# jambo6/online-neural-cdes

Hardware: AMD Instinct MI355X
Metric: solved integration steps/sec (fwd+adjoint) (higher is better)
Workload: dtype f32; 1 GPU; BASELINE cfg2: rectilinear interpolation, rk4 step 1, B=4096 per GPU (global 4096), raw L=200 -> T=399 knots, C=20, H=HH=32, nl=3; step = forward + adjoint backward + Adam; global_batch=4096, seq_len=200, parallelism=dp1

## Files before the change

### online-neural-cdes_amd/csrc/ncde_coop.h

```cpp
#pragma once
#include "ncde_bf3.h"
#include "ncde_common.h"

#define COOP_NRT 5
#define COOP_RPM (4 * COOP_NRT)
#define COOP_NCH 4
#define COOP_SPIN_LIMIT (1 << 22)

namespace {

typedef unsigned u32x2c __attribute__((ext_vector_type(2)));
typedef _Float16 h16x4 __attribute__((ext_vector_type(4)));

struct CoopDims {
    int H, C, dlast, M, G;
    __host__ __device__ int xl() const { return dlast * 16; }
    __host__ __device__ int off_as() const { return xl(); }
    __host__ __device__ int off_dx() const { return off_as() + H * 16; }
    __host__ __device__ int off_sc() const { return off_dx() + C * 16; }
    __host__ __device__ int off_ko() const { return off_sc() + 64; }
    __host__ __device__ int off_part() const { return off_ko() + H * 16; }
    __host__ __device__ long long per_tile() const { return (long long)off_part() + (long long)M * dlast * 16; }
    __host__ __device__ long long per_tile_fwd() const { return (long long)off_part(); }
};

__device__ __forceinline__ __amdgpu_buffer_rsrc_t coop_rsrc(const void* p) {
    return __builtin_amdgcn_make_buffer_rsrc(const_cast<void*>(p), 0, 0x7ffffffc, 0x00020000);
}
__device__ __forceinline__ void coop_st16(__amdgpu_buffer_rsrc_t r, float* base, bool same, long long float_off, u32x4 v) {
    if (same) *reinterpret_cast<u32x4*>(base + float_off) = v;
    else __builtin_amdgcn_raw_buffer_store_b128(v, r, (int)(float_off * 4), 0, 16);
}
__device__ __forceinline__ void coop_st4(__amdgpu_buffer_rsrc_t r, float* base, bool same, long long float_off, float v) {
    if (same) base[float_off] = v;
    else __builtin_amdgcn_raw_buffer_store_b32(__float_as_uint(v), r, (int)(float_off * 4), 0, 16);
}
__device__ __forceinline__ u32x4 coop_ld16(__amdgpu_buffer_rsrc_t r, long long float_off) {
    return __builtin_amdgcn_raw_buffer_load_b128(r, (int)(float_off * 4), 0, 16);
}
__device__ __forceinline__ float coop_ld4(__amdgpu_buffer_rsrc_t r, long long float_off) {
    return __uint_as_float(__builtin_amdgcn_raw_buffer_load_b32(r, (int)(float_off * 4), 0, 16));
}
__device__ __forceinline__ f32x4 coop_ld16f(__amdgpu_buffer_rsrc_t r, long long float_off) {
    return __builtin_bit_cast(f32x4, coop_ld16(r, float_off));
}

__device__ __forceinline__ float coop_pow2_scale(float m) {
    if (!(m > 0.0f) || !(m < 3.0e38f)) return 1.0f;
    int e = (int)((__float_as_uint(m) >> 23) & 255u) - 126;
    e = e < -100 ? -100 : (e > 100 ? 100 : e);
    return __uint_as_float((unsigned)(127 - e) << 23);
}
__device__ __forceinline__ float coop_pow2_inv(float s) { return __uint_as_float((254u - ((__float_as_uint(s) >> 23) & 255u)) << 23); }

struct CoopSync {
    unsigned* words;
    int G;
    unsigned* status;
    unsigned spin;
};
__device__ __forceinline__ void coop_give_up(const CoopSync& sy) {
    __hip_atomic_store(sy.words + sy.G, 1u, __ATOMIC_RELAXED, __HIP_MEMORY_SCOPE_AGENT);
    __hip_atomic_store(sy.status, 1u, __ATOMIC_RELAXED, __HIP_MEMORY_SCOPE_AGENT);
}
__host__ __device__ inline int coop_sync_words(int G, int n_tiles) { return 2 * G + 1 + n_tiles; }
__device__ __forceinline__ void coop_arrive(const CoopSync& sy, int g) {
    __hip_atomic_fetch_add(sy.words + g, 1u, __ATOMIC_RELAXED, __HIP_MEMORY_SCOPE_AGENT);
}
__device__ __forceinline__ bool coop_wait(const CoopSync& sy, int g, unsigned target, int* flag_lds, int tid) {
    if (tid == 0) {
        int ok = 1;
        unsigned spins = 0;
// ... 146 lines not shown
```

### online-neural-cdes_amd/csrc/ncde_dwo2.hip

```cpp
#include "ncde_common.h"
#include "ncde_bf3.h"
#define NCDE_COOP_NO_KERNELS
#include "ncde_coop.h"
#include "ncde_dwo2.h"

template <int NRT>
__device__ __forceinline__ void dwo_h2_body(const KArgs& a, int n_sc, int n_st, float* gpartB) {
    extern __shared__ __attribute__((aligned(16))) float lds[];
    constexpr int dlast = 128, PK = 8, NCH = 4, NWV = 16 / NRT;
    const int tid = threadIdx.x, lane = tid & 63;
    const int wave = __builtin_amdgcn_readfirstlane(tid >> 6);
    const int li = lane & 15, lk = lane >> 4;
    const int C = a.C, H = a.H, ncq = C >> 2;
    const int n_pair = n_st >> 1, parts = a.dw2_parts, nrg = gridDim.x / parts;
    int bx_, by_;
    if ((parts & 7) == 0) {
        const int xcd = blockIdx.x & 7, slot = blockIdx.x >> 3;
        by_ = xcd * (parts >> 3) + slot / nrg;
        bx_ = slot % nrg;
    } else {
        by_ = blockIdx.x / nrg;
        bx_ = blockIdx.x % nrg;
    }
    const int bx = __builtin_amdgcn_readfirstlane(bx_), by = __builtin_amdgcn_readfirstlane(by_);
    const int nRC = H >> 4, nRD = (C + 15) >> 4;
    const int oXP = 2 * 2048, oRC = oXP + 4096, oRD = oRC + 2 * nRC * 256, oS = oRD + 2 * nRD * 256, per_buf = oS + 2 * 256;
    int hb[NRT], cq[NRT];
    u32x4 W[NRT][NCH][2];
    float bias[NRT];
    f32x4 gW[NRT][PK];
    float gb[NRT];
#pragma unroll
    for (int q = 0; q < NRT; ++q) {
        const int rt = (bx * NWV + wave) * NRT + q;
        hb[q] = rt / ncq;
        cq[q] = rt - hb[q] * ncq;
        const int mem = rt / COOP_RPM, rw = (rt % COOP_RPM) / COOP_NRT, qq = rt % COOP_NRT;
        const unsigned* wp = a.coop_img + (long long)mem * (coop_p_words() + coop_t_words()) + rw * (40 * 64 * 4);
#pragma unroll
        for (int c = 0; c < NCH; ++c)
#pragma unroll
            for (int pc = 0; pc < 2; ++pc) W[q][c][pc] = *reinterpret_cast<const u32x4*>(wp + ((((qq * 4 + c) * 2 + pc) * 64) + lane) * 4);
        bias[q] = a.bo[(4 * hb[q] + (li >> 2)) * C + 4 * cq[q] + (li & 3)];
#pragma unroll
        for (int jt = 0; jt < PK; ++jt) gW[q][jt] = (f32x4){0.f, 0.f, 0.f, 0.f};
        gb[q] = 0.0f;
    }
    const float sigma = coop_pow2_scale(__uint_as_float(*a.win_max)), inv_sigma = coop_pow2_inv(sigma);
    const int my_n = by < n_pair ? (n_pair - by + parts - 1) / parts : 0;
    typedef const __attribute__((address_space(1))) void* gptr_t;
    typedef __attribute__((address_space(3))) void* lptr_t;
    const int n_chunk = 2 * 8 + 16 + 2 * nRC + 2 * nRD + 2;
#ifndef DW2_NIW
#define DW2_NIW 4
#endif
    constexpr int NIW = DW2_NIW < NWV ? DW2_NIW : NWV;
    constexpr int NSLOT = (60 + NIW - 1) / NIW;
    long long s_const[NSLOT];
    int s_sc[NSLOT], s_pr[NSLOT], s_lds[NSLOT];
#pragma unroll
    for (int j = 0; j < NSLOT; ++j) {
        int k = wave + NIW * j;
        if (k >= n_chunk) k = wave < NIW ? wave : 0;
        long long cst;
        int ssc, spr, sl;
        if (k < 16) { cst = (long long)(k >> 3) * 2048 + (k & 7) * 256; ssc = n_st * 2048; spr = 2 * 2048; sl = k * 256; }
        else if ((k -= 16) < 16) { cst = (a.recB - a.recA) + (long long)k * 256; ssc = n_pair * 4096; spr = 4096; sl = oXP + k * 256; }
        else if ((k -= 16) < 2 * nRC) { const int t2 = k >= nRC ? 1 : 0, kk = k - t2 * nRC; cst = (a.recC - a.recA) + (long long)t2 * (H * 16) + kk * 256; ssc = n_st * H * 16; spr = 2 * H * 16; sl = oRC + k * 256; }
        else if ((k -= 2 * nRC) < 2 * nRD) { const int t2 = k >= nRD ? 1 : 0, kk = k - t2 * nRD; cst = (a.recD - a.recA) + (long long)t2 * (C * 16) + kk * 256; ssc = n_st * C * 16; spr = 2 * C * 16; sl = oRD + k * 256; }
        else { k -= 2 * nRD; cst = (a.recS - a.recA) + (long long)k * 32; ssc = n_st * 32; spr = 64; sl = oS + k * 256; }
        s_const[j] = cst; s_sc[j] = ssc; s_pr[j] = spr; s_lds[j] = sl;
    }
    const int my_n_ = by < n_pair ? (n_pair - by + parts - 1) / parts : 0;
    long long s_off[NSLOT];
    int s_dpr[NSLOT], s_dsc[NSLOT];
#pragma unroll
    for (int j = 0; j < NSLOT; ++j) {
        s_off[j] = s_const[j] + (long long)by * s_pr[j];
        s_dpr[j] = parts * s_pr[j];
        s_dsc[j] = s_sc[j] - (my_n_ - 1) * parts * s_pr[j];
    }
    auto issue = [&](bool wrap, int buf) {
        if (wave >= NIW) return;
#pragma unroll
        for (int j = 0; j < NSLOT; ++j) {
            __builtin_amdgcn_global_load_lds((gptr_t)(a.recA + s_off[j] + lane * 4), (lptr_t)(lds + buf * per_buf + s_lds[j]), 16, 0, 0);
            s_off[j] += wrap ? s_dsc[j] : s_dpr[j];
        }
    };
#ifdef NCDE_DW2_PROF
    unsigned long long dprof[5] = {0, 0, 0, 0, 0}, dlast_ = __builtin_readcyclecounter();
#define DW2_TICK(k) { const unsigned long long n_ = __builtin_readcyclecounter(); dprof[k] += n_ - dlast_; dlast_ = n_; }
#else
#define DW2_TICK(k)
#endif
    u32x4 Ap[NRT][2];
    auto p_and_epilogue = [&](int buf, int lane, int li, int lk) {
        const float* B_ = lds + buf * per_buf;
        const unsigned* XS = reinterpret_cast<const unsigned*>(B_);
        auto ldx = [&](int t2, int c, int pc) { return *reinterpret_cast<const u32x4*>(XS + t2 * 2048 + ((c * 2 + pc) * 64 + lane) * 4); };
        constexpr bool AHEAD = NRT == 4;
        u32x4 nx0, nx1;
        if constexpr (AHEAD) { nx0 = ldx(0, 0, 0); nx1 = ldx(0, 0, 1); }
#pragma unroll
        for (int t2 = 0; t2 < 2; ++t2) {
            const float* S_ = B_ + oS + t2 * 256;
            const f32x4 isx4 = *reinterpret_cast<const f32x4*>(S_ + 4 * lk);
            f32x4 isx2;
#pragma unroll
            for (int r = 0; r < 4; ++r) isx2[r] = isx4[r] * NCDE_TANH_PRESCALE;
            const float fT = sigma * S_[17];
            auto lda = [&](int i) { return *reinterpret_cast<const f32x4*>(B_ + oRC + t2 * nRC * 256 + (4 * hb[i] + (li >> 2)) * 16 + 4 * lk); };
            auto ldd = [&](int i) { return *reinterpret_cast<const f32x4*>(B_ + oRD + t2 * nRD * 256 + (4 * cq[i] + (li & 3)) * 16 + 4 * lk); };
            f32x4 na4, nd4;
            if constexpr (AHEAD) { na4 = lda(0); nd4 = ldd(0); }
            f32x4 pm[NRT], px[NRT];
#pragma unroll
            for (int i = 0; i < NRT; ++i) {
#pragma unroll
                for (int r = 0; r < 4; ++r) pm[i][r] = bias[i] * coop_pow2_inv(isx4[r]);
                px[i] = (f32x4){0.f, 0.f, 0.f, 0.f};
            }
#pragma unroll
            for (int c = 0; c < NCH; ++c) {
                u32x4 x0, x1;
                if constexpr (AHEAD) {
                    x0 = nx0; x1 = nx1;
                    if (c + 1 < NCH) { nx0 = ldx(t2, c + 1, 0); nx1 = ldx(t2, c + 1, 1); }
                    else if (t2 == 0) { nx0 = ldx(1, 0, 0); nx1 = ldx(1, 0, 1); }
                } else { x0 = ldx(t2, c, 0); x1 = ldx(t2, c, 1); }
#pragma unroll
                for (int i = 0; i < NRT; ++i) px[i] = mfma_h(x0, W[i][c][1], px[i]);
#pragma unroll
                for (int i = 0; i < NRT; ++i) pm[i] = mfma_h(x0, W[i][c][0], pm[i]);
#pragma unroll
                for (int i = 0; i < NRT; ++i) px[i] = mfma_h(x1, W[i][c][0], px[i]);
            }
#pragma unroll
            for (int i = 0; i < NRT; ++i) {
                const f32x4 pc = h2_combine(pm[i], px[i]);
                f32x4 a4, d4;
                if constexpr (AHEAD) {
                    a4 = na4; d4 = nd4;
                    if (i + 1 < NRT) { na4 = lda(i + 1); nd4 = ldd(i + 1); }
                } else { a4 = lda(i); d4 = ldd(i); }
                float dps[4];
#pragma unroll
                for (int r = 0; r < 4; ++r) {
                    const float th = tanh_prescaled(pc[r] * isx2[r]);
                    const float dp = (a4[r] * d4[r]) * (1.0f - th * th);
                    gb[i] += dp;
                    dps[r] = dp * fT;
                }
                unsigned h0, l0, h1, l1;
                coop_split2(dps[0], dps[1], h0, l0);
                coop_split2(dps[2], dps[3], h1, l1);
                Ap[i][0][2 * t2] = h0; Ap[i][0][2 * t2 + 1] = h1;
                Ap[i][1][2 * t2] = l0; Ap[i][1][2 * t2 + 1] = l1;
            }
        }
    };
    auto dwo_products = [&](int buf, int lane) {
        const unsigned* XP = reinterpret_cast<const unsigned*>(lds + buf * per_buf + oXP);
        constexpr bool AHEAD = NRT == 4;
        auto ldb = [&](int jt, int pc) { return *reinterpret_cast<const u32x4*>(XP + ((jt * 2 + pc) * 64 + lane) * 4); };
        u32x4 nb0, nb1;
        if constexpr (AHEAD) { nb0 = ldb(0, 0); nb1 = ldb(0, 1); }
        f32x4 ptx[NRT];
#pragma unroll
        for (int jt = 0; jt < PK; ++jt) {
            u32x4 b0, b1;
            if constexpr (AHEAD) {
                b0 = nb0; b1 = nb1;
                if (jt + 1 < PK) { nb0 = ldb(jt + 1, 0); nb1 = ldb(jt + 1, 1); }
            } else { b0 = ldb(jt, 0); b1 = ldb(jt, 1); }
            f32x4 tx[NRT];
#pragma unroll
            for (int i = 0; i < NRT; ++i) tx[i] = mfma_h(Ap[i][0], b1, (f32x4){0.f, 0.f, 0.f, 0.f});
#pragma unroll
            for (int i = 0; i < NRT; ++i) gW[i][jt] = mfma_h(Ap[i][0], b0, gW[i][jt]);
#pragma unroll
            for (int i = 0; i < NRT; ++i) tx[i] = mfma_h(Ap[i][1], b0, tx[i]);
            if (jt > 0) {
#pragma unroll
                for (int i = 0; i < NRT; ++i) gW[i][jt - 1] = h2_combine(gW[i][jt - 1], ptx[i]);
            }
#pragma unroll
            for (int i = 0; i < NRT; ++i) ptx[i] = tx[i];
        }
#pragma unroll
        for (int i = 0; i < NRT; ++i) gW[i][PK - 1] = h2_combine(gW[i][PK - 1], ptx[i]);
    };
    if (my_n > 0 && n_sc > 0) {
        const int nq = n_sc * my_n;
        int k_n = 0;
        issue(k_n + 1 == my_n, 0);
        if (++k_n == my_n) k_n = 0;
        asm volatile("s_waitcnt vmcnt(0)" ::: "memory");
        __syncthreads();
        for (int q = 0; q < nq; ++q) {
            const int buf = q & 1;
            if (q + 1 < nq) {
                issue(k_n + 1 == my_n, buf ^ 1);
                if (++k_n == my_n) k_n = 0;
            }
            __builtin_amdgcn_sched_barrier(0);
            DW2_TICK(0)
            int t_ = tid;
            asm volatile("" : "+v"(t_));
            const int lane_ = t_ & 63, li_ = t_ & 15, lk_ = (t_ >> 4) & 3;
            p_and_epilogue(buf, lane_, li_, lk_);
            DW2_TICK(1)
            dwo_products(buf, lane_);
            DW2_TICK(2)
            __builtin_amdgcn_sched_barrier(0);
            asm volatile("s_waitcnt vmcnt(0)" ::: "memory");
            DW2_TICK(3)
            __syncthreads();
            DW2_TICK(4)
        }
#ifdef NCDE_DW2_PROF
        if (lane == 0)
            for (int k = 0; k < 5; ++k) a.grad_z0[((long long)blockIdx.x * NWV + wave) * 8 + k] = (float)dprof[k] / (float)nq;
#endif
    }
    const long long wo_sz = (long long)H * C * dlast, theta_o = wo_sz + (long long)H * C;
    float* gp = gpartB + (long long)by * theta_o;
#pragma unroll
    for (int q = 0; q < NRT; ++q) {
#pragma unroll
        for (int jt = 0; jt < PK; ++jt)
#pragma unroll
            for (int r = 0; r < 4; ++r) {
                float* dst = gp + ((long long)(4 * hb[q] + lk) * C + 4 * cq[q] + r) * dlast + 16 * jt + li;
                const float v = gW[q][jt][r] * inv_sigma;
                *dst = a.dw2_accum ? *dst + v : v;
            }
        float v = gb[q];
        v += __shfl_xor(v, 16, 64); v += __shfl_xor(v, 32, 64);
        if (lk == 0) {
            float* dst = gp + wo_sz + (4 * hb[q] + (li >> 2)) * C + 4 * cq[q] + (li & 3);
            *dst = a.dw2_accum ? *dst + v : v;
        }
    }
}

extern "C" __global__ __launch_bounds__(512) void ncde_dwo_h2(KArgs a, int n_sc, int n_st, float* gpartB) { dwo_h2_body<2>(a, n_sc, n_st, gpartB); }
```

### online-neural-cdes_amd/csrc/ncde_tiled.hip

```cpp
#include <type_traits>
#include "ncde_common.h"
#include "ncde_bf3.h"
#include "ncde_host.h"
#include "ncde_tiled.h"
#include "ncde_coop.h"
#include "ncde_dwo2.h"

#define TL_NW 8
#define TL_THREADS (64 * TL_NW)
#define TL_EMAX 16

namespace {

template <int NS, int NT, bool QUINTIC = true>
__device__ __forceinline__ void tl_load_dx(const KArgs& a, int b0, int idx, float frac, float kdt, float* DX, int tid) {
    constexpr int NSP = NS * 16;
    const int C = a.C, Cc = a.Cc;
    for (int e = tid; e < NSP * C; e += NT) {
        const int s = e / C, c = e - s * C;
        const int b = b0 + s;
        float v = 0.0f;
        if (b < a.B && c < Cc) {
            const float* p = a.coeffs + (long long)b * a.cs_b + (long long)idx * a.cs_t;
            if (a.interp == NCDE_INTERP_LINEAR) {
// ... 676 lines not shown
            const float v = live ? a.z0[(long long)b * a.Hr + u] : 0.0f;
            y0[q] = v;
            YS[e] = v;
            if (live) a.out[((long long)b * a.n_out) * a.Hr + u] = v;
        }
    }
    const int S = n_stages(a.method);
    const int dlast = a.dout[a.n_layers - 1];
    const int nkb_o = dlast >> 4;
    Panel<RESH ? RESH : 1> wf[2];
    f32x4 bfv[2];
    if constexpr (RESH != 0) {
        const int li = lane & 15, lk = lane >> 4;
        int l1 = 0;
        for (int l = 1; l < a.n_layers; ++l)
            if (a.W[l] != a.W[0]) { l1 = l; break; }
#pragma unroll
        for (int sl = 0; sl < 2; ++sl) {
            const int l = sl == 0 ? 0 : l1;
            const int tw = wave < RESH ? wave : 0;
            wf[sl] = tl_load_panel<RESH ? RESH : 1>(a.W[l] + (long long)(16 * tw + li) * (16 * RESH) + 4 * lk, 0);
            bfv[sl] = *reinterpret_cast<const f32x4*>(a.b[l] + 16 * tw + 4 * lk);
        }
    }
    int cur_idx = -1;
    const bool planned = a.plan != nullptr;
    if (planned && !plan_header_ok(a, S)) return;
    const int n_steps = planned ? a.n_steps_fwd : a.T - 1;
    const int* pout = planned ? a.plan + plan_off_out(S, a.n_steps_fwd) : nullptr;
    int sc = 0;
#ifdef NCDE_TL_PROF
    unsigned long long fprof[8] = {0, 0, 0, 0, 0, 0, 0, 0}, flast = __builtin_readcyclecounter();
    unsigned long long kprof[3] = {0, 0, 0}, klast = 0;
#endif
    for (int n = 0; n < n_steps; ++n) {
        const int* pstep = planned ? a.plan + plan_off_fwd() + n * plan_step_words(S) : nullptr;
        const float dt = planned ? __int_as_float(pstep[0]) : 1.0f;
        for (int j = 0; j < S; ++j, ++sc) {
            const StageDesc sd = planned ? plan_stage(pstep, j) : default_stage(a.method, (float)n + stage_offset(a.method, j), a.n_pieces);
            const int idx = sd.idx;
            bool dx_new = false;
            if constexpr (DIRECT != 0) {
                tl_load_cin<NS, NT>(a, b0, sd, a.field_input == NCDE_INPUT_EVALUATE, YS, H, tid);
            } else if (a.interp != NCDE_INTERP_LINEAR || idx != cur_idx) {
                tl_load_dx<NS, NT, COOP == 0>(a, b0, idx, sd.frac, sd.kdt, DX, tid);
                cur_idx = idx;
                dx_new = true;
            }
            __syncthreads();
            if constexpr (COOP != 0) {
                if (dx_new) {
                    const long long my_base = (long long)blockIdx.x * cd.per_tile_fwd();
                    for (int e = tid; e < a.C * NSP / 4; e += NT) coop_st16(crs, a.coop_x, c_same, my_base + cd.off_dx() + e * 4, *reinterpret_cast<const u32x4*>(DX + e * 4));
                }
            }
            if (a.stages) {
                const int Hr = a.Hr;
                float* rec = a.stages + ((long long)(n * S + j) * (a.Brec ? a.Brec : a.B) + b0) * Hr;
                for (int e = tid; e < NSP * Hr; e += NT) {
                    const int s = e / Hr, u = e - s * Hr;
                    if (b0 + s < a.B) rec[e] = YS[((u >> 2) * NSP + s) * 4 + (u & 3)];
                }
            }
            FW_TICK(0)
            const float* in = YS;
            for (int l = 0; l < a.n_layers; ++l) {
                float* outb = (l & 1) ? ACT1 : ACT0;
                if constexpr (RESH != 0) {
                    if (wave < RESH) {
                        const int li = lane & 15, lk = lane >> 4;
                        const bool s0 = a.W[l] == a.W[0];
                        f32x4 acc[1];
                        acc[0] = s0 ? bfv[0] : bfv[1];
                        if (s0) tl_mma_panel<1, RESH ? RESH : 1>(wf[0], in, 0, li, lk, acc);
                        else tl_mma_panel<1, RESH ? RESH : 1>(wf[1], in, 0, li, lk, acc);
                        f32x4 o;
#pragma unroll
                        for (int r = 0; r < 4; ++r) o[r] = relu_dev(acc[0][r]);
                        *reinterpret_cast<f32x4*>(outb + ((4 * wave + lk) * NSP + li) * 4) = o;
                        if constexpr (BF != 0) {
                            if (l == a.n_layers - 1) {
                                typedef unsigned u32x2 __attribute__((ext_vector_type(2)));
                                if constexpr (BF == 2) {
                                    unsigned h0, l0, h1, l1;
                                    split_pair_h(o[0], o[1], h0, l0, mx);
                                    split_pair_h(o[2], o[3], h1, l1, mx);
                                    unsigned* dst = XB + ((((wave >> 1) * 2) * 4 + 2 * (wave & 1) + (lk >> 1)) * 16 + li) * 4 + 2 * (lk & 1);
                                    *reinterpret_cast<u32x2*>(dst) = (u32x2){h0, h1};
                                    *reinterpret_cast<u32x2*>(dst + 256) = (u32x2){l0, l1};
                                } else {
                                    unsigned h0, m0, l0, h1, m1, l1;
                                    split_pair(o[0], o[1], h0, m0, l0);
                                    split_pair(o[2], o[3], h1, m1, l1);
                                    unsigned* dst = XB + ((((wave >> 1) * 3) * 4 + 2 * (wave & 1) + (lk >> 1)) * 16 + li) * 4 + 2 * (lk & 1);
                                    *reinterpret_cast<u32x2*>(dst) = (u32x2){h0, h1};
                                    *reinterpret_cast<u32x2*>(dst + 256) = (u32x2){m0, m1};
                                    *reinterpret_cast<u32x2*>(dst + 512) = (u32x2){l0, l1};
                                }
                            }
                        }
                    }
                } else {
                    const TlW wr_ = tl_wref(lds, DIRECT != 0 ? a.tres[l] : 0, a.W[l], a.b[l], a.dout[l], a.din[l]);
                    if constexpr (COOP != 0)
                        tl_dense_relu<NS, NWV, 0, 0, 4>(wr_.W, wr_.b, a.dout[l], a.din[l], in, outb, wave, lane, nullptr, wr_.ld);
                    else if constexpr (BF == 2)
                        tl_dense_relu<NS, NWV, 0, 1>(wr_.W, wr_.b, a.dout[l], a.din[l], in, outb, wave, lane,
                                                     l == a.n_layers - 1 ? XB : nullptr, wr_.ld, &mx);
                    else
                        tl_dense_relu<NS, NWV>(wr_.W, wr_.b, a.dout[l], a.din[l], in, outb, wave, lane,
                                               (BF != 0 && l == a.n_layers - 1) ? XB : nullptr, wr_.ld);
                }
                __syncthreads();
                in = outb;
            }
            FW_TICK(1)
            float* KG = in == ACT0 ? ACT1 : ACT0;
            if constexpr (DIRECT != 0) {
                const TlW wo_ = tl_wref(lds, a.tres_o, a.Wo, a.bo, H, dlast);
                tl_dense_relu<NS, NWV, 1>(wo_.W, wo_.b, H, dlast, in, KO, wave, lane, nullptr, wo_.ld);
                if constexpr (GATED != 0) {
                    const TlW wg_ = tl_wref(lds, a.tres_g, a.Wg, a.bg, H, dlast);
                    tl_dense_relu<NS, NWV, 2>(wg_.W, wg_.b, H, dlast, in, KG, wave, lane, nullptr, wg_.ld);
                }
            } else
            if constexpr (COOP != 0) {
                const int li = lane & 15, lk = lane >> 4, C = a.C;
                const long long my_base = (long long)blockIdx.x * cd.per_tile_fwd();
                const unsigned bar1 = (2u * (unsigned)sc + 1u) * (unsigned)cd.M, bar2 = bar1 + (unsigned)cd.M;
                {
                    float mxl = 0.0f;
                    for (int e = tid; e < 128 * NSP; e += NT) mxl = fmaxf(mxl, fabsf(in[e]));
                    mxl = fmaxf(mxl, __shfl_xor(mxl, 1, 64)); mxl = fmaxf(mxl, __shfl_xor(mxl, 2, 64));
                    if ((lane & 3) == 0) CMX[wave * 16 + ((lane >> 2) & 15)] = mxl;
                }
                __syncthreads();
                if (tid < 16) {
                    float m_ = 0.0f;
#pragma unroll
                    for (int wv = 0; wv < 8; ++wv) m_ = fmaxf(m_, CMX[wv * 16 + tid]);
                    const float sx = coop_pow2_scale(m_), isx = coop_pow2_inv(sx) * a.coop_scale[1];
                    CSG[tid] = sx; CSG[16 + tid] = isx;
                    coop_st4(crs, a.coop_x, c_same, my_base + cd.off_sc() + tid, sx); coop_st4(crs, a.coop_x, c_same, my_base + cd.off_sc() + 16 + tid, isx);
                }
                __syncthreads();
                if (wave < 4) {
                    const int c = wave, ub = 32 * c + 8 * lk;
                    const f32x4 v0 = *reinterpret_cast<const f32x4*>(in + (((ub >> 2)) * NSP + li) * 4);
                    const f32x4 v1 = *reinterpret_cast<const f32x4*>(in + (((ub >> 2) + 1) * NSP + li) * 4);
                    const float sx = CSG[li];
                    unsigned h[4], l[4];
                    coop_split2(v0[0] * sx, v0[1] * sx, h[0], l[0]); coop_split2(v0[2] * sx, v0[3] * sx, h[1], l[1]);
                    coop_split2(v1[0] * sx, v1[1] * sx, h[2], l[2]); coop_split2(v1[2] * sx, v1[3] * sx, h[3], l[3]);
                    coop_st16(crs, a.coop_x, c_same, my_base + ((c * 2 + 0) * 64 + lane) * 4, (u32x4){h[0], h[1], h[2], h[3]});
                    coop_st16(crs, a.coop_x, c_same, my_base + ((c * 2 + 1) * 64 + lane) * 4, (u32x4){l[0], l[1], l[2], l[3]});
                }
                asm volatile("s_waitcnt vmcnt(0)" ::: "memory");
                __syncthreads();
                if (tid == 0 && !(a.coop_inject != 0 && blockIdx.x == 1 && sc == 0)) coop_arrive(csy, c_grp);
                FW_TICK(2)
                auto poison = [&]() {
                    const float qnan = __builtin_nanf("");
                    for (long long e = tid; e < (long long)NSP * a.n_out * a.Hr; e += NT)
                        if (b0 + (int)(e / ((long long)a.n_out * a.Hr)) < a.B) a.out[(long long)b0 * a.n_out * a.Hr + e] = qnan;
                };
                if (!coop_wait(csy, c_grp, bar1, CFL, tid)) { poison(); return; }
                FW_TICK(3)
                const int ncq = C >> 2, jh = COOP_RPM / ncq, wph = 4 / jh;
                const int rw = wave & 3, half_w = wave >> 2;
                const int cq0 = (c_mem * COOP_RPM + rw * COOP_NRT) % ncq;
                const int n_dx4 = C * NSP / 4, n_it = cd.M / 2;
                typedef const __attribute__((address_space(1))) void* gptr_t;
                typedef __attribute__((address_space(3))) void* lptr_t;
                const int n_dxw = (n_dx4 + 63) >> 6;
                auto stage_load = [&](int it_, int buf, int tid) {
                    const int wv = __builtin_amdgcn_readfirstlane(tid >> 6), w64 = wv * 64;
#pragma unroll
                    for (int hf = 0; hf < 2; ++hf) {
                        const float* src = a.coop_x + (long long)(c_grp + cd.G * (2 * it_ + hf)) * cd.per_tile_fwd();
                        __builtin_amdgcn_global_load_lds((gptr_t)(src + tid * 4), (lptr_t)(CBX + (buf * 2 + hf) * 2048 + w64 * 4), 16, 0, 16);
                        if (wv < n_dxw) __builtin_amdgcn_global_load_lds((gptr_t)(src + cd.off_dx() + tid * 4), (lptr_t)(CDX + (buf * 2 + hf) * 1280 + w64 * 4), 16, 0, 16);
                        else if (wv == 6 && tid < 400)
                            __builtin_amdgcn_global_load_lds((gptr_t)(src + cd.off_sc() + (tid - 384) * 4), (lptr_t)(CSC + (buf * 2 + hf) * 64), 16, 0, 16);
                    }
                };
                stage_load(0, 0, tid);
                asm volatile("s_waitcnt vmcnt(0)" ::: "memory");
                __syncthreads();
                const int tid_outer = tid;
#ifdef NCDE_TL_PROF
                klast = __builtin_readcyclecounter();
#endif
                for (int it = 0; it <= n_it; ++it) {
                    int tid = tid_outer;
                    asm volatile("" : "+v"(tid));
                    const int lane = tid & 63, li = tid & 15, lk = (tid >> 4) & 3;
                    const int buf = it & 1;
                    if (it + 1 < n_it) stage_load(it + 1, buf ^ 1, tid);
                    if (it < n_it) {
                        const float* bxs = CBX + (buf * 2 + half_w) * 2048;
                        const float isx = CSC[(buf * 2 + half_w) * 64 + 16 + li];
                        const float sxw = coop_pow2_inv(isx);
                        const float isx2 = isx * NCDE_TANH_PRESCALE;
                        float kk = 0.0f;
                        auto wfr = [&](int k) -> u32x4 {
                            if (k < FWD_KREG) return cw.f[k];
                            return *reinterpret_cast<const u32x4*>(CWL + ((rw * (40 - FWD_KREG) + (k - FWD_KREG)) * 64 + lane) * 4);
                        };
                        auto p_batch = [&](auto q0c, auto nqc) {
                            constexpr int Q0 = decltype(q0c)::value, NQ = decltype(nqc)::value;
                            f32x4 pm[NQ], px[NQ];
#pragma unroll
                            for (int i = 0; i < NQ; ++i) {
                                const f32x4 bsv = *reinterpret_cast<const f32x4*>(CBO + ((rw * COOP_NRT + Q0 + i) * 4 + lk) * 4);
#pragma unroll
                                for (int r = 0; r < 4; ++r) pm[i][r] = bsv[r] * sxw;
                                px[i] = (f32x4){0.f, 0.f, 0.f, 0.f};
                            }
                            u32x4 b0_ = *reinterpret_cast<const u32x4*>(bxs + lane * 4), b1_ = *reinterpret_cast<const u32x4*>(bxs + (64 + lane) * 4);
#pragma unroll
                            for (int c = 0; c < COOP_NCH; ++c) {
                                const u32x4 c0_ = b0_, c1_ = b1_;
                                if (c + 1 < COOP_NCH) {
                                    b0_ = *reinterpret_cast<const u32x4*>(bxs + (((c + 1) * 2 + 0) * 64 + lane) * 4);
                                    b1_ = *reinterpret_cast<const u32x4*>(bxs + (((c + 1) * 2 + 1) * 64 + lane) * 4);
                                }
#pragma unroll
                                for (int i = 0; i < NQ; ++i) pm[i] = mfma_h(wfr(((Q0 + i) * 4 + c) * 2 + 0), c0_, pm[i]);
#pragma unroll
                                for (int i = 0; i < NQ; ++i) px[i] = mfma_h(wfr(((Q0 + i) * 4 + c) * 2 + 1), c0_, px[i]);
#pragma unroll
                                for (int i = 0; i < NQ; ++i) px[i] = mfma_h(wfr(((Q0 + i) * 4 + c) * 2 + 0), c1_, px[i]);
                            }
#pragma unroll
                            for (int i = 0; i < NQ; ++i) {
                                const f32x4 pc4 = h2_combine(pm[i], px[i]);
                                const f32x4 dxv = *reinterpret_cast<const f32x4*>(CDX + (buf * 2 + half_w) * 1280 + ((cq0 + Q0 + i) * NSP + li) * 4);
#pragma unroll
                                for (int r = 0; r < 4; ++r) kk = fmaf(tanh_prescaled(pc4[r] * isx2), dxv[r], kk);
                            }
                        };
                        if ((wave & 1) == 0) {
                            p_batch(std::integral_constant<int, 0>{}, std::integral_constant<int, 3>{});
                            p_batch(std::integral_constant<int, 3>{}, std::integral_constant<int, 2>{});
                        } else {
                            p_batch(std::integral_constant<int, 3>{}, std::integral_constant<int, 2>{});
                            p_batch(std::integral_constant<int, 0>{}, std::integral_constant<int, 3>{});
                        }
                        CKX[(buf * 8 + wave) * 64 + lane] = kk;
                    }
                    if (it >= 1 && tid < 2 * 64 * jh) {
                        const int hf = tid / (64 * jh), hl = (tid >> 6) % jh, ln = tid & 63, pb = buf ^ 1;
                        float ksum = 0.0f;
                        for (int wv = hl * wph; wv < (hl + 1) * wph; ++wv) ksum += CKX[(pb * 8 + 4 * hf + wv) * 64 + ln];
                        const long long tb = (long long)(c_grp + cd.G * (2 * (it - 1) + hf)) * cd.per_tile_fwd();
                        coop_st4(crs, a.coop_x, c_same, tb + cd.off_ko() + ((c_mem * jh + hl) * NSP + (ln & 15)) * 4 + (ln >> 4), ksum);
                    }
#ifdef NCDE_TL_PROF
                    { const unsigned long long n_ = __builtin_readcyclecounter(); kprof[0] += n_ - klast; klast = n_; }
#endif
                    if (it + 1 < n_it) asm volatile("s_waitcnt vmcnt(0)" ::: "memory");
#ifdef NCDE_TL_PROF
                    { const unsigned long long n_ = __builtin_readcyclecounter(); kprof[1] += n_ - klast; klast = n_; }
#endif
                    __syncthreads();
#ifdef NCDE_TL_PROF
                    { const unsigned long long n_ = __builtin_readcyclecounter(); kprof[2] += n_ - klast; klast = n_; }
#endif
                }
                asm volatile("s_waitcnt vmcnt(0)" ::: "memory");
                __syncthreads();
                FW_TICK(4)
                if (tid == 0) coop_arrive(csy, c_grp);
                if (!coop_wait(csy, c_grp, bar2, CFL, tid)) { poison(); return; }
                FW_TICK(5)
                for (int e4 = tid * 4; e4 < HS; e4 += NT * 4) *reinterpret_cast<f32x4*>(KO + e4) = coop_ld16f(crs, my_base + cd.off_ko() + e4);
            } else
            if constexpr (BF == 2) {
                switch (nkb_o) {
                    case 8: tl_output_h2<4, NWV, GATED>(a, XB, DX, KO, wave, lane); break;
                    case 4: tl_output_h2<2, NWV, GATED>(a, XB, DX, KO, wave, lane); break;
                    default: tl_output_h2<1, NWV, GATED>(a, XB, DX, KO, wave, lane); break;
                }
            } else if constexpr (BF != 0) {
                switch (nkb_o) {
                    case 8: tl_output_bf<4, NWV, GATED>(a, XB, DX, KO, wave, lane); break;
                    case 4: tl_output_bf<2, NWV, GATED>(a, XB, DX, KO, wave, lane); break;
                    default: tl_output_bf<1, NWV, GATED>(a, XB, DX, KO, wave, lane); break;
                }
            } else
            switch (nkb_o) {
                case 8: tl_output_whole<NS, 8, NWV, GATED>(a, in, DX, KO, wave, lane); break;
                case 4: tl_output_whole<NS, 4, NWV, GATED>(a, in, DX, KO, wave, lane); break;
                case 2: tl_output_whole<NS, 2, NWV, GATED>(a, in, DX, KO, wave, lane); break;
                case 1: tl_output_whole<NS, 1, NWV, GATED>(a, in, DX, KO, wave, lane); break;
// ... 444 lines not shown
        }
    }

    Panel<PK> wf[2];
    f32x4 bfv[2];
    float wb[2][4 * PK];
    WoTile<PK> wo[2];
    if constexpr (RES != 0) {
        const int li = lane & 15, lk = lane >> 4;
        int l1 = 0;
        for (int l = 1; l < L; ++l)
            if (a.gW_off[l] != a.gW_off[0]) { l1 = l; break; }
        const int K = dlast;
#pragma unroll
        for (int sl = 0; sl < 2; ++sl) {
            const int l = sl == 0 ? 0 : l1;
            const int tw = wave < PK ? wave : 0;
            wf[sl] = tl_load_panel<PK>(a.W[l] + (long long)(16 * tw + li) * K + 4 * lk, 0);
            bfv[sl] = *reinterpret_cast<const f32x4*>(a.b[l] + 16 * tw + 4 * lk);
#pragma unroll
            for (int kb = 0; kb < PK; ++kb)
#pragma unroll
                for (int e = 0; e < 4; ++e) wb[sl][4 * kb + e] = a.W[l][(long long)(16 * kb + 4 * lk + e) * K + 16 * tw + li];
        }
        if constexpr (RES == 1) {
            const int nhb = H >> 2, ncq = C >> 2;
#pragma unroll
            for (int q = 0; q < 2; ++q) {
                int hb = wave + NWV * (q / ncq), cq = q % ncq;
                if (hb >= nhb) { hb = 0; cq = 0; }
                wo[q].P = tl_load_panel<PK>(a.Wo + (long long)((4 * hb + (li >> 2)) * C + 4 * cq + (li & 3)) * dlast + 4 * lk, 0);
                wo[q].bias = *reinterpret_cast<const f32x4*>(a.bo + (4 * hb + lk) * C + 4 * cq);
            }
        }
    }

    CoopWeights cw;
    CoopDims cd{};
    CoopSync csy{};
    __amdgpu_buffer_rsrc_t crs = coop_rsrc(a.coop_x);
    int c_grp = 0, c_mem = 0, c_hbw = 0;
    bool c_same = false;
    float* const CDP = SC;
    float* const CBX = CDP + 2 * 10 * 2 * 64 * 4;
    float* const CDX = CBX + 2 * 8 * 64 * 4;
    float* const CAS = CDX + 2 * 80 * 16;
    float* const CSC = CAS + 2 * 256;
    float* const CKX = CSC + 2 * 64;
    float* const CIS = CKX + 2 * 4 * 64;
    int* const CFL = reinterpret_cast<int*>(CIS + 2 * 16);
    float* const CBO = reinterpret_cast<float*>(XBA) + 2048;
    float* const CMX = CDP;
    float* const CSG = CDP + 3 * 8 * 16;
    if constexpr (COOP != 0) {
        cd.H = H; cd.C = C; cd.dlast = dlast; cd.M = a.coop_M; cd.G = a.coop_G;
        csy.words = a.coop_sync; csy.G = a.coop_G; csy.status = a.coop_status; csy.spin = a.coop_spin;
        c_grp = blockIdx.x % a.coop_G;
        c_mem = blockIdx.x / a.coop_G;
        c_hbw = (c_mem * COOP_RPM + (wave & 3) * COOP_NRT) / (C >> 2);
        coop_load_weights<0, COOP_PIN>(cw, a.coop_img, c_mem, wave, lane);
        const int same = coop_same_xcd(csy, c_grp, c_mem, a.coop_M, (int)gridDim.x, CFL, tid);
        if (same < 0) return;
        c_same = same != 0;
    }

    constexpr int DXMAXC = NWV == 8 ? 80 : 160;
    constexpr int DXE = (NSP * DXMAXC + NT - 1) / NT, YSE = TL_EADJ;
    float dxn[DXE], ysn[YSE];
    const bool wide_c = C > DXMAXC;
    StageDesc sdn;
    const float* recn = nullptr;
    auto stage_desc = [&](int n, int j) {
        if (planned) return plan_stage(step_of(n), disc ? S - 1 - j : j);
        return default_stage(a.method, disc ? (float)(n - 1) + stage_offset(a.method, S - 1 - j) : -(-(float)n + stage_offset(a.method, j)), a.n_pieces);
    };
    auto dx_value = [&](int e, const StageDesc& sd) {
        const int idx = sd.idx;
        const float frac = sd.frac, kdt = sd.kdt;
        float v = 0.0f;
        const int s = e / C, c = e - s * C, b = b0 + s;
        const int Cc = a.Cc;
        if (b < a.B && c < Cc) {
            const float* cp = a.coeffs + (long long)b * a.cs_b + (long long)idx * a.cs_t;
            const bool value = DIRECT != 0 && a.field_input == NCDE_INPUT_EVALUATE;
            if (a.interp == NCDE_INTERP_LINEAR) {
                v = cp[a.cs_t + c] - cp[c];
                if (value) v = cp[c] + (frac * v) / kdt;
                else if (kdt != 1.0f) v = v / kdt;
            } else if (COOP == 0 && a.interp == NCDE_INTERP_QUINTIC) {
                v = quintic_eval(cp + c, Cc, frac, value);
            } else {
                const float bb = cp[Cc + c], cc = cp[2 * Cc + c], dd = cp[3 * Cc + c];
                if (value) {
                    float inner = 0.5f * cc + (dd * frac) / 3.0f;
                    inner = bb + inner * frac;
                    v = cp[c] + inner * frac;
                } else {
                    const float inner = cc + dd * frac;
                    v = bb + inner * frac;
                }
            }
        }
        return v;
    };
    auto prefetch = [&](int n, int j) {
        sdn = stage_desc(n, j);
// ... 138 lines not shown
                    }
                    for (int e = tid; e < H * NSP; e += NT) {
                        const int hh = e >> 4, s = e & 15;
                        rc[e] = w * AS[((hh >> 2) * NSP + s) * 4 + (hh & 3)];
                    }
                    for (int e = tid; e < C * NSP; e += NT) rd[e] = DX[e];
            };
            if constexpr (DIRECT != 0) {
                float* DPT = G0;
                float* SG = SC;
                const TlW wo_ = tl_wref(lds, a.tres_o, a.Wo, a.bo, H, dlast);
                const TlW wg_ = tl_wref(lds, GATED != 0 ? a.tres_g : 0, a.Wg, a.bg, H, dlast);
                tl_dense_relu<1, NWV, 1>(wo_.W, wo_.b, H, dlast, in, KOY, wave, lane, nullptr, wo_.ld);
                if constexpr (GATED != 0) tl_dense_relu<1, NWV, 2>(wg_.W, wg_.b, H, dlast, in, SG, wave, lane, nullptr, wg_.ld);
                __syncthreads();
                for (int e = tid; e < HS; e += NT) {
                    const float th = KOY[e], dm = AS[e];
                    if constexpr (GATED != 0) {
                        const float sg = SG[e];
                        KOY[e] = sg * th;
                        DPT[e] = (dm * sg) * (1.0f - th * th);
                        SG[e] = (dm * th) * (sg * (1.0f - sg));
                    } else {
                        DPT[e] = dm * (1.0f - th * th);
                    }
                }
                __syncthreads();
                if (w != 0.0f) {
                    tl_dw_acc<NWV, TL_DWT>(DPT, in, H, dlast, w, dwo, wave, lane);
                    if constexpr (GATED != 0) tl_dw_acc<NWV, TL_DWT>(SG, in, H, dlast, w, dwg, wave, lane);
                    if (tid < H) {
                        float sum = 0.0f, sumg = 0.0f;
#pragma unroll
                        for (int s = 0; s < NSP; ++s) {
                            sum += DPT[((tid >> 2) * NSP + s) * 4 + (tid & 3)];
                            if constexpr (GATED != 0) sumg += SG[((tid >> 2) * NSP + s) * 4 + (tid & 3)];
                        }
                        dbo += w * sum;
                        dbg += w * sumg;
                    }
                }
                tl_hidden_bwd<NWV>(wo_.W, H, dlast, DPT, in, true, G1, wave, lane, GATED != 0 ? wg_.W : nullptr, GATED != 0 ? SG : nullptr, wo_.ld);
                __syncthreads();
            } else {
                if constexpr (COOP != 0) {
                    const int li = lane & 15, lk = lane >> 4;
                    const long long my_base = (long long)blockIdx.x * cd.per_tile();
                    const unsigned bar1 = (2u * (unsigned)sc + 1u) * (unsigned)cd.M, bar2 = bar1 + (unsigned)cd.M;
                    {
                        float mx = 0.0f, ma = 0.0f, md = 0.0f;
                        for (int e = tid; e < dlast * NSP; e += NT) mx = fmaxf(mx, fabsf(in[e]));
                        for (int e = tid; e < HS; e += NT) ma = fmaxf(ma, fabsf(AS[e]));
                        for (int e = tid; e < C * NSP; e += NT) md = fmaxf(md, fabsf(DX[e]));
                        mx = fmaxf(mx, __shfl_xor(mx, 1, 64)); mx = fmaxf(mx, __shfl_xor(mx, 2, 64));
                        ma = fmaxf(ma, __shfl_xor(ma, 1, 64)); ma = fmaxf(ma, __shfl_xor(ma, 2, 64));
                        md = fmaxf(md, __shfl_xor(md, 1, 64)); md = fmaxf(md, __shfl_xor(md, 2, 64));
                        if ((lane & 3) == 0) {
                            const int s_ = (lane >> 2) & 15;
                            CMX[(0 * 8 + wave) * 16 + s_] = mx; CMX[(1 * 8 + wave) * 16 + s_] = ma; CMX[(2 * 8 + wave) * 16 + s_] = md;
                        }
                    }
                    __syncthreads();
                    if (tid < 16) {
                        float m3[3];
#pragma unroll
                        for (int k = 0; k < 3; ++k) {
                            float m_ = 0.0f;
#pragma unroll
                            for (int wv = 0; wv < 8; ++wv) m_ = fmaxf(m_, CMX[(k * 8 + wv) * 16 + tid]);
                            m3[k] = m_;
                        }
                        const float sw_inv = a.coop_scale[1];
                        const float sx = coop_pow2_scale(m3[0]), sd = coop_pow2_scale(m3[1] * m3[2]);
                        const float isx = coop_pow2_inv(sx) * sw_inv, isd = coop_pow2_inv(sd) * sw_inv;
                        CSG[tid] = sx; CSG[16 + tid] = isx; CSG[32 + tid] = sd; CSG[48 + tid] = isd;
                        coop_st4(crs, a.coop_x, c_same, my_base + cd.off_sc() + tid, sx); coop_st4(crs, a.coop_x, c_same, my_base + cd.off_sc() + 16 + tid, isx);
                        coop_st4(crs, a.coop_x, c_same, my_base + cd.off_sc() + 32 + tid, sd); coop_st4(crs, a.coop_x, c_same, my_base + cd.off_sc() + 48 + tid, isd);
                        float mt = m3[0], bt = fabsf(w) * (m3[1] * m3[2]);
#pragma unroll
                        for (int o = 8; o > 0; o >>= 1) { mt = fmaxf(mt, __shfl_xor(mt, o, 64)); bt = fmaxf(bt, __shfl_xor(bt, o, 64)); }
                        const float uT = coop_pow2_scale(mt), iuT = coop_pow2_inv(uT);
                        float* rs = a.recS + ((long long)sc * n_st + blockIdx.x) * 32;
                        rs[tid] = isx;
                        if (tid == 0) {
                            CSG[64] = uT;
                            rs[16] = uT; rs[17] = iuT;
                            const float bq = bt * iuT;
                            if (bq > 0.0f && bq < 3.0e38f) atomicMax(a.win_max, __float_as_uint(bq));
                        }
                    }
                    __syncthreads();
                    if (wave < 4) {
                        const int c = wave, ub = 32 * c + 8 * lk;
                        const f32x4 v0 = *reinterpret_cast<const f32x4*>(in + (((ub >> 2)) * NSP + li) * 4);
                        const f32x4 v1 = *reinterpret_cast<const f32x4*>(in + (((ub >> 2) + 1) * NSP + li) * 4);
                        const float sx = CSG[li];
                        unsigned h[4], l[4];
                        coop_split2(v0[0] * sx, v0[1] * sx, h[0], l[0]); coop_split2(v0[2] * sx, v0[3] * sx, h[1], l[1]);
                        coop_split2(v1[0] * sx, v1[1] * sx, h[2], l[2]); coop_split2(v1[2] * sx, v1[3] * sx, h[3], l[3]);
                        coop_st16(crs, a.coop_x, c_same, my_base + ((c * 2 + 0) * 64 + lane) * 4, (u32x4){h[0], h[1], h[2], h[3]});
                        coop_st16(crs, a.coop_x, c_same, my_base + ((c * 2 + 1) * 64 + lane) * 4, (u32x4){l[0], l[1], l[2], l[3]});
                    }
                    {
                        for (int e = tid; e < HS / 4; e += NT) coop_st16(crs, a.coop_x, c_same, my_base + cd.off_as() + e * 4, *reinterpret_cast<const u32x4*>(AS + e * 4));
                        for (int e = tid; e < C * NSP / 4; e += NT) coop_st16(crs, a.coop_x, c_same, my_base + cd.off_dx() + e * 4, *reinterpret_cast<const u32x4*>(DX + e * 4));
                    }
                    asm volatile("s_waitcnt vmcnt(0)" ::: "memory");
                    __syncthreads();
                    if (tid == 0 && !(a.coop_inject != 0 && blockIdx.x == 1 && sc == 0 && a.resume == 0)) coop_arrive(csy, c_grp);
                    TL_TICK(8)
                    coop_load_weights<COOP_PIN, 40>(cw, a.coop_img, c_mem, wave, lane);
                    {
                        const long long tile = (long long)sc * n_st + blockIdx.x;
                        if (wave < 4) {
                            const int c = wave, ub = 32 * c + 8 * lk;
                            const f32x4 v0 = *reinterpret_cast<const f32x4*>(in + (((ub >> 2)) * NSP + li) * 4);
                            const f32x4 v1 = *reinterpret_cast<const f32x4*>(in + (((ub >> 2) + 1) * NSP + li) * 4);
                            const float sx = CSG[li];
                            unsigned h[4], l[4];
                            coop_split2(v0[0] * sx, v0[1] * sx, h[0], l[0]); coop_split2(v0[2] * sx, v0[3] * sx, h[1], l[1]);
                            coop_split2(v1[0] * sx, v1[1] * sx, h[2], l[2]); coop_split2(v1[2] * sx, v1[3] * sx, h[3], l[3]);
                            unsigned* ra = reinterpret_cast<unsigned*>(a.recA) + tile * 2048;
                            *reinterpret_cast<u32x4*>(ra + ((c * 2 + 0) * 64 + lane) * 4) = (u32x4){h[0], h[1], h[2], h[3]};
                            *reinterpret_cast<u32x4*>(ra + ((c * 2 + 1) * 64 + lane) * 4) = (u32x4){l[0], l[1], l[2], l[3]};
                        }
                        {
                            const float uT = CSG[64];
                            unsigned* rbp = reinterpret_cast<unsigned*>(a.recB) + ((long long)sc * (n_st >> 1) + (blockIdx.x >> 1)) * 4096;
                            const int half = blockIdx.x & 1;
                            for (int e = tid; e < 128 * 4; e += NT) {
                                const int k = e >> 2, kg = e & 3, ln = (k & 15) + 16 * kg;
                                float v[4];
#pragma unroll
                                for (int q = 0; q < 4; ++q) v[q] = in[((k >> 2) * NSP + 4 * kg + q) * 4 + (k & 3)] * uT;
                                unsigned h0, l0, h1, l1;
                                coop_split2(v[0], v[1], h0, l0);
                                coop_split2(v[2], v[3], h1, l1);
                                unsigned* dst = rbp + (((k >> 4) * 2) * 64 + ln) * 4 + 2 * half;
                                *reinterpret_cast<u32x2c*>(dst) = (u32x2c){h0, h1};
// ... 1706 lines not shown
```

Measured before the change: 195.1 million sample-steps/s.

## Skip MFMA work for zero channel quads when dx is narrow (rectilinear)

Detects at runtime whether the control-path increments are nonzero only in the first channel quad, which is typical for rectilinear interpolation where only one channel changes per knot. It writes a per-tile 'wide' flag into the cooperative buffer and the recS records, and the forward p_batch and dwo2 backward stages then run only the row tile holding channel quad 0. The goal is to cut MFMA and epilogue work on these sparse steps. In exchange it adds a scan of the dx values, an extra barrier, repurposes the sx scale slot for the flag by dropping the sx store, and depends on the flag being exactly zero for correctness.

```diff
diff --git a/online-neural-cdes_amd/csrc/ncde_coop.h b/online-neural-cdes_amd/csrc/ncde_coop.h
--- a/online-neural-cdes_amd/csrc/ncde_coop.h
+++ b/online-neural-cdes_amd/csrc/ncde_coop.h
@@ -5,6 +5,8 @@
 #define COOP_NRT 5
 #define COOP_RPM (4 * COOP_NRT)
 #define COOP_NCH 4
+#define COOP_WIDE 0
+#define COOP_RECS_WIDE 18
 #define COOP_SPIN_LIMIT (1 << 22)
 
 namespace {
@@ -18,6 +20,7 @@
     __host__ __device__ int off_as() const { return xl(); }
     __host__ __device__ int off_dx() const { return off_as() + H * 16; }
     __host__ __device__ int off_sc() const { return off_dx() + C * 16; }
+    __host__ __device__ int off_wide() const { return off_sc() + COOP_WIDE; }
     __host__ __device__ int off_ko() const { return off_sc() + 64; }
     __host__ __device__ int off_part() const { return off_ko() + H * 16; }
     __host__ __device__ long long per_tile() const { return (long long)off_part() + (long long)M * dlast * 16; }
diff --git a/online-neural-cdes_amd/csrc/ncde_dwo2.hip b/online-neural-cdes_amd/csrc/ncde_dwo2.hip
--- a/online-neural-cdes_amd/csrc/ncde_dwo2.hip
+++ b/online-neural-cdes_amd/csrc/ncde_dwo2.hip
@@ -3,6 +3,15 @@
 #define NCDE_COOP_NO_KERNELS
 #include "ncde_coop.h"
 #include "ncde_dwo2.h"
+#include <type_traits>
+
+template <int I, int N, class F>
+__device__ __forceinline__ void dwo_h2_one_of(int q0, F& f) {
+    if constexpr (I < N) {
+        if (q0 == I) f(std::integral_constant<int, (1 << I)>{});
+        else dwo_h2_one_of<I + 1, N>(q0, f);
+    }
+}
 
 template <int NRT>
 __device__ __forceinline__ void dwo_h2_body(const KArgs& a, int n_sc, int n_st, float* gpartB) {
@@ -94,12 +103,18 @@
 #else
 #define DW2_TICK(k)
 #endif
+    constexpr int FULL = (1 << NRT) - 1;
+    static_assert(NRT < 5, "a wave's row tiles must hold at most one of channel quad 0");
+    int q0 = -1;
+#pragma unroll
+    for (int q = 0; q < NRT; ++q) q0 = cq[q] == 0 ? q : q0;
     u32x4 Ap[NRT][2];
-    auto p_and_epilogue = [&](int buf, int lane, int li, int lk) {
+    auto p_and_epilogue = [&](auto mkc, int buf, int lane, int li, int lk) {
+        constexpr int MK = decltype(mkc)::value;
         const float* B_ = lds + buf * per_buf;
         const unsigned* XS = reinterpret_cast<const unsigned*>(B_);
         auto ldx = [&](int t2, int c, int pc) { return *reinterpret_cast<const u32x4*>(XS + t2 * 2048 + ((c * 2 + pc) * 64 + lane) * 4); };
-        constexpr bool AHEAD = NRT == 4;
+        constexpr bool AHEAD = NRT == 4 && MK == FULL;
         u32x4 nx0, nx1;
         if constexpr (AHEAD) { nx0 = ldx(0, 0, 0); nx1 = ldx(0, 0, 1); }
 #pragma unroll
@@ -117,6 +132,7 @@
             f32x4 pm[NRT], px[NRT];
 #pragma unroll
             for (int i = 0; i < NRT; ++i) {
+                if (((MK >> i) & 1) == 0) continue;
 #pragma unroll
                 for (int r = 0; r < 4; ++r) pm[i][r] = bias[i] * coop_pow2_inv(isx4[r]);
                 px[i] = (f32x4){0.f, 0.f, 0.f, 0.f};
@@ -130,14 +146,15 @@
                     else if (t2 == 0) { nx0 = ldx(1, 0, 0); nx1 = ldx(1, 0, 1); }
                 } else { x0 = ldx(t2, c, 0); x1 = ldx(t2, c, 1); }
 #pragma unroll
-                for (int i = 0; i < NRT; ++i) px[i] = mfma_h(x0, W[i][c][1], px[i]);
-#pragma unroll
-                for (int i = 0; i < NRT; ++i) pm[i] = mfma_h(x0, W[i][c][0], pm[i]);
-#pragma unroll
-                for (int i = 0; i < NRT; ++i) px[i] = mfma_h(x1, W[i][c][0], px[i]);
+                for (int i = 0; i < NRT; ++i) if ((MK >> i) & 1) px[i] = mfma_h(x0, W[i][c][1], px[i]);
+#pragma unroll
+                for (int i = 0; i < NRT; ++i) if ((MK >> i) & 1) pm[i] = mfma_h(x0, W[i][c][0], pm[i]);
+#pragma unroll
+                for (int i = 0; i < NRT; ++i) if ((MK >> i) & 1) px[i] = mfma_h(x1, W[i][c][0], px[i]);
             }
 #pragma unroll
             for (int i = 0; i < NRT; ++i) {
+                if (((MK >> i) & 1) == 0) continue;
                 const f32x4 pc = h2_combine(pm[i], px[i]);
                 f32x4 a4, d4;
                 if constexpr (AHEAD) {
@@ -160,7 +177,8 @@
             }
         }
     };
-    auto dwo_products = [&](int buf, int lane) {
+    auto dwo_products = [&](auto mkc, int buf, int lane) {
+        constexpr int MK = decltype(mkc)::value;
         const unsigned* XP = reinterpret_cast<const unsigned*>(lds + buf * per_buf + oXP);
         constexpr bool AHEAD = NRT == 4;
         auto ldb = [&](int jt, int pc) { return *reinterpret_cast<const u32x4*>(XP + ((jt * 2 + pc) * 64 + lane) * 4); };
@@ -176,20 +194,20 @@
             } else { b0 = ldb(jt, 0); b1 = ldb(jt, 1); }
             f32x4 tx[NRT];
 #pragma unroll
-            for (int i = 0; i < NRT; ++i) tx[i] = mfma_h(Ap[i][0], b1, (f32x4){0.f, 0.f, 0.f, 0.f});
-#pragma unroll
-            for (int i = 0; i < NRT; ++i) gW[i][jt] = mfma_h(Ap[i][0], b0, gW[i][jt]);
-#pragma unroll
-            for (int i = 0; i < NRT; ++i) tx[i] = mfma_h(Ap[i][1], b0, tx[i]);
+            for (int i = 0; i < NRT; ++i) if ((MK >> i) & 1) tx[i] = mfma_h(Ap[i][0], b1, (f32x4){0.f, 0.f, 0.f, 0.f});
+#pragma unroll
+            for (int i = 0; i < NRT; ++i) if ((MK >> i) & 1) gW[i][jt] = mfma_h(Ap[i][0], b0, gW[i][jt]);
+#pragma unroll
+            for (int i = 0; i < NRT; ++i) if ((MK >> i) & 1) tx[i] = mfma_h(Ap[i][1], b0, tx[i]);
             if (jt > 0) {
 #pragma unroll
-                for (int i = 0; i < NRT; ++i) gW[i][jt - 1] = h2_combine(gW[i][jt - 1], ptx[i]);
-            }
-#pragma unroll
-            for (int i = 0; i < NRT; ++i) ptx[i] = tx[i];
-        }
-#pragma unroll
-        for (int i = 0; i < NRT; ++i) gW[i][PK - 1] = h2_combine(gW[i][PK - 1], ptx[i]);
+                for (int i = 0; i < NRT; ++i) if ((MK >> i) & 1) gW[i][jt - 1] = h2_combine(gW[i][jt - 1], ptx[i]);
+            }
+#pragma unroll
+            for (int i = 0; i < NRT; ++i) if ((MK >> i) & 1) ptx[i] = tx[i];
+        }
+#pragma unroll
+        for (int i = 0; i < NRT; ++i) if ((MK >> i) & 1) gW[i][PK - 1] = h2_combine(gW[i][PK - 1], ptx[i]);
     };
     if (my_n > 0 && n_sc > 0) {
         const int nq = n_sc * my_n;
@@ -209,10 +227,17 @@
             int t_ = tid;
             asm volatile("" : "+v"(t_));
             const int lane_ = t_ & 63, li_ = t_ & 15, lk_ = (t_ >> 4) & 3;
-            p_and_epilogue(buf, lane_, li_, lk_);
-            DW2_TICK(1)
-            dwo_products(buf, lane_);
-            DW2_TICK(2)
+            const float* S_ = lds + buf * per_buf + oS;
+            const bool narrow = a.dense_channels == 0 &&
+                (__builtin_amdgcn_readfirstlane(__float_as_uint(S_[COOP_RECS_WIDE])) | __builtin_amdgcn_readfirstlane(__float_as_uint(S_[256 + COOP_RECS_WIDE]))) == 0u;
+            auto pair_stage = [&](auto mkc) {
+                p_and_epilogue(mkc, buf, lane_, li_, lk_);
+                DW2_TICK(1)
+                dwo_products(mkc, buf, lane_);
+                DW2_TICK(2)
+            };
+            if (!narrow) pair_stage(std::integral_constant<int, FULL>{});
+            else dwo_h2_one_of<0, NRT>(q0, pair_stage);
             __builtin_amdgcn_sched_barrier(0);
             asm volatile("s_waitcnt vmcnt(0)" ::: "memory");
             DW2_TICK(3)
diff --git a/online-neural-cdes_amd/csrc/ncde_tiled.hip b/online-neural-cdes_amd/csrc/ncde_tiled.hip
--- a/online-neural-cdes_amd/csrc/ncde_tiled.hip
+++ b/online-neural-cdes_amd/csrc/ncde_tiled.hip
@@ -752,6 +752,17 @@
                 if (dx_new) {
                     const long long my_base = (long long)blockIdx.x * cd.per_tile_fwd();
                     for (int e = tid; e < a.C * NSP / 4; e += NT) coop_st16(crs, a.coop_x, c_same, my_base + cd.off_dx() + e * 4, *reinterpret_cast<const u32x4*>(DX + e * 4));
+                    bool nz = false;
+                    for (int e = 64 + tid; e < a.C * NSP; e += NT) nz = nz || !(DX[e] == 0.0f);
+                    const bool wnz = __builtin_amdgcn_ballot_w64(nz) != 0;
+                    if (lane == 0) CMX[wave * 16] = wnz ? 1.0f : 0.0f;
+                    __syncthreads();
+                    if (tid == 0) {
+                        float wd = 0.0f;
+#pragma unroll
+                        for (int wv = 0; wv < 8; ++wv) wd = fmaxf(wd, CMX[wv * 16]);
+                        coop_st4(crs, a.coop_x, c_same, my_base + cd.off_wide(), wd);
+                    }
                 }
             }
             if (a.stages) {
@@ -841,7 +852,7 @@
                     for (int wv = 0; wv < 8; ++wv) m_ = fmaxf(m_, CMX[wv * 16 + tid]);
                     const float sx = coop_pow2_scale(m_), isx = coop_pow2_inv(sx) * a.coop_scale[1];
                     CSG[tid] = sx; CSG[16 + tid] = isx;
-                    coop_st4(crs, a.coop_x, c_same, my_base + cd.off_sc() + tid, sx); coop_st4(crs, a.coop_x, c_same, my_base + cd.off_sc() + 16 + tid, isx);
+                    coop_st4(crs, a.coop_x, c_same, my_base + cd.off_sc() + 16 + tid, isx);
                 }
                 __syncthreads();
                 if (wave < 4) {
@@ -940,7 +951,11 @@
                                 for (int r = 0; r < 4; ++r) kk = fmaf(tanh_prescaled(pc4[r] * isx2), dxv[r], kk);
                             }
                         };
-                        if ((wave & 1) == 0) {
+                        const bool narrow = a.dense_channels == 0 &&
+                            __builtin_amdgcn_readfirstlane(__float_as_uint(CSC[(buf * 2 + half_w) * 64 + COOP_WIDE])) == 0u;
+                        if (narrow) {
+                            if (cq0 == 0) p_batch(std::integral_constant<int, 0>{}, std::integral_constant<int, 1>{});
+                        } else if ((wave & 1) == 0) {
                             p_batch(std::integral_constant<int, 0>{}, std::integral_constant<int, 3>{});
                             p_batch(std::integral_constant<int, 3>{}, std::integral_constant<int, 2>{});
                         } else {
@@ -1491,6 +1506,7 @@
     float* const CBO = reinterpret_cast<float*>(XBA) + 2048;
     float* const CMX = CDP;
     float* const CSG = CDP + 3 * 8 * 16;
+    float* const CWD = CSG + 80;
     if constexpr (COOP != 0) {
         cd.H = H; cd.C = C; cd.dlast = dlast; cd.M = a.coop_M; cd.G = a.coop_G;
         csy.words = a.coop_sync; csy.G = a.coop_G; csy.status = a.coop_status; csy.spin = a.coop_spin;
@@ -1735,6 +1751,10 @@
                         for (int e = tid; e < dlast * NSP; e += NT) mx = fmaxf(mx, fabsf(in[e]));
                         for (int e = tid; e < HS; e += NT) ma = fmaxf(ma, fabsf(AS[e]));
                         for (int e = tid; e < C * NSP; e += NT) md = fmaxf(md, fabsf(DX[e]));
+                        bool nz = false;
+                        for (int e = 64 + tid; e < C * NSP; e += NT) nz = nz || !(DX[e] == 0.0f);
+                        const bool wnz = __builtin_amdgcn_ballot_w64(nz) != 0;
+                        if (lane == 0) CWD[wave] = wnz ? 1.0f : 0.0f;
                         mx = fmaxf(mx, __shfl_xor(mx, 1, 64)); mx = fmaxf(mx, __shfl_xor(mx, 2, 64));
                         ma = fmaxf(ma, __shfl_xor(ma, 1, 64)); ma = fmaxf(ma, __shfl_xor(ma, 2, 64));
                         md = fmaxf(md, __shfl_xor(md, 1, 64)); md = fmaxf(md, __shfl_xor(md, 2, 64));
@@ -1768,6 +1788,10 @@
                         if (tid == 0) {
                             CSG[64] = uT;
                             rs[16] = uT; rs[17] = iuT;
+                            float wd = 0.0f;
+#pragma unroll
+                            for (int wv = 0; wv < 8; ++wv) wd = fmaxf(wd, CWD[wv]);
+                            rs[COOP_RECS_WIDE] = wd;
                             const float bq = bt * iuT;
                             if (bq > 0.0f && bq < 3.0e38f) atomicMax(a.win_max, __float_as_uint(bq));
                         }
```

Result: no change. 194.9 million sample-steps/s (-0.1%).
